# carlobaldassi/GaussDCA.jl

Hardware: AMD Instinct MI355X
Metric: end-to-end gDCA sec + achieved Cholesky TFLOP/s, N=500 M=50k q=21 (higher is better)
Workload: dtype f64

## Files before the change

gaussdca.jl_amd/csrc/gdca_api.hip:

```cpp
#include <algorithm>
#include <ctype.h>
#include <math.h>
#include <stdio.h>
#include <stdlib.h>
#include <string.h>
#include <strings.h>

#include "gdca_internal.h"
#include "gdca_launch.h"

#define MAX_EV 1024
#define N_SCRATCH 10

struct gdca_buf {
    void *p;
    size_t cap;
};

struct gdca_gate {
    hipEvent_t ev[4];
    int next, last, armed, refs;
    hipStream_t batch_stream;
};

// ... 609 lines not shown

static gdca_status member_error(gdca_ctx *lead, gdca_ctx *m, int k, gdca_status st)
{
    if (k > 0 && m != lead && m->err[0]) {
        char msg[sizeof(lead->err)];
        snprintf(msg, sizeof(msg), "member %d: %.400s", k, m->err);
        memcpy(lead->err, msg, sizeof(msg));
    }
    return st;
}

static gdca_status upload_done(gdca_ctx *ctx)
{
    HIPCHK(hipEventRecord(ctx->ev_upload, ctx->stream));
    HIPCHK(hipEventSynchronize(ctx->ev_upload));
    return GDCA_OK;
}

static double inverse_flops_model(double n)
{
    return (n * n * n / 3.0 + n * n / 2.0 + n / 6.0) + (2.0 * n * n * n / 3.0 + n * n / 2.0 + 5.0 * n / 6.0);
}

static int round_up(int x, int m)
{
    return (x + m - 1) / m * m;
}

static gdca_status weights_stage(gdca_ctx *ctx, const int8_t *Zd, int N, int M, int q, double theta_in, int fixed_thresh,
                                 bool want_theta_only, int mark_after_theta)
{
    hipStream_t s = ctx->stream;
    gdca_dev_scalars *sc = (gdca_dev_scalars *)ctx->sc.p;
    CHK(ensure(ctx, ctx->hist, (size_t)N * 32 * sizeof(uint32_t)));
    if (fixed_thresh >= 0) {
        gdca_launch_set_thresh(s, sc, fixed_thresh);
    } else {
        if (theta_in < 0.0) {
            gdca_fill_async(s, ctx->hist.p, 0, (size_t)N * 32 * sizeof(uint32_t));
            gdca_launch_column_hist(s, Zd, (uint32_t *)ctx->hist.p, N, M);
        }
        gdca_launch_theta_finalize(s, (const uint32_t *)ctx->hist.p, N, M, theta_in, sc);
    }
    CHK(check_launch(ctx, "theta"));
    if (mark_after_theta >= 0) CHK(mark(ctx, mark_after_theta));
    if (want_theta_only) return GDCA_OK;

    const int Mt = (M + GDCA_HTILE - 1) / GDCA_HTILE;
    CHK(ensure(ctx, ctx->Zb, gdca_bitplane_bytes(N, M)));
    CHK(ensure(ctx, ctx->hcnt, (size_t)Mt * GDCA_HTILE * sizeof(int32_t)));
    if (!ctx->tune.force_fallback && ctx->tune.hamming_mode != 0) CHK(ensure(ctx, ctx->hcand, gdca_hamming_cand_cap(M) * 8));
    const bool fp4 = !ctx->tune.force_fallback && ctx->tune.hamming_mode == 2;
    if (fp4) CHK(ensure(ctx, ctx->himg, gdca_fp4_image_bytes(N, M)));
    CHK(ensure(ctx, ctx->nk, (size_t)M * sizeof(int32_t)));
    CHK(ensure(ctx, ctx->W, (size_t)M * sizeof(double)));
    CHK(ensure(ctx, ctx->Wfix, (size_t)M * sizeof(unsigned long long)));
    gdca_fill_async(s, ctx->hcnt.p, 0, (size_t)Mt * GDCA_HTILE * sizeof(int32_t));
    gdca_launch_bitplane_pack(s, Zd, (uint32_t *)ctx->Zb.p, N, M, q, sc);
    if (ctx->tune.force_fallback)
        gdca_launch_hamming_fallback(s, Zd, (int32_t *)ctx->hcnt.p, N, M, sc);
    else
        gdca_launch_hamming(s, (const uint32_t *)ctx->Zb.p, Zd, (int32_t *)ctx->hcnt.p, N, M, sc, ctx->tune.hamming_mode, ctx->hcand.p, fp4 ? ctx->himg.p : nullptr);
    gdca_launch_weights(s, (const int32_t *)ctx->hcnt.p, M, gdca_fix_shift(M), (int32_t *)ctx->nk.p,
                        (double *)ctx->W.p, (unsigned long long *)ctx->Wfix.p);
    gdca_launch_meff(s, (const double *)ctx->W.p, M, sc);
    return check_launch(ctx, "weights");
}

static bool norm1_settled(const gdca_ctx *ctx, int N, int q, double pc)
{
    const double pi_cap = (1.0 - pc) + pc / (double)q;
    return pc > 0.0 && 2.0 * (double)N * pi_cap * (double)q * (double)q / pc <= ctx->tune.refine_cond && ctx->tune.refine != 1;
}

static gdca_status tally_stage(gdca_ctx *ctx, const int8_t *Zd, int N, int M, int q, const double *Meff_dev, double pc,
                               int mode, double *Pi_true_out, double *out, size_t ld, bool want_norm1 = false)
{
    hipStream_t s = ctx->stream;
    const int sdim = q - 1, n = N * sdim;
    const int shift = gdca_fix_shift(M);
    const int TJ = gdca_tally_tj(q, ctx->tune.tally_tj);
    const bool skip = gdca_tally_skip(q, TJ, ctx->tune.tally_skip, M);
    const size_t keep_list = (size_t)N * M * sizeof(uint32_t);
    if (skip) CHK(ensure(ctx, ctx->keep, keep_list + (size_t)N * sizeof(int) + N));
    CHK(ensure(ctx, ctx->Zt, (size_t)N * M));
    CHK(ensure(ctx, ctx->Zp, (size_t)round_up(N, 64) * M + 64));
    CHK(ensure(ctx, ctx->Pifix, (size_t)N * 32 * sizeof(unsigned long long)));
    CHK(ensure(ctx, ctx->Pipc, (size_t)n * sizeof(double)));
    gdca_launch_transpose_i8(s, Zd, (int8_t *)ctx->Zt.p, N, M);
    gdca_launch_colblock(s, Zd, (int8_t *)ctx->Zp.p, N, M, TJ);
    gdca_fill_async(s, ctx->Pifix.p, 0, (size_t)N * 32 * sizeof(unsigned long long));
    gdca_launch_pi_tally(s, Zd, (const unsigned long long *)ctx->Wfix.p, (unsigned long long *)ctx->Pifix.p, N, M, q,
                         (gdca_dev_scalars *)ctx->sc.p);
    gdca_launch_pi_finalize(s, (const unsigned long long *)ctx->Pifix.p, N, q, shift, Meff_dev, pc, Pi_true_out,
                            (double *)ctx->Pipc.p, want_norm1 ? &((gdca_dev_scalars *)ctx->sc.p)->pi_max : nullptr);
    const bool tm = want_norm1 && ctx->timing && ctx->n_ev >= 18;
    if (tm) CHK(mark(ctx, 9));
    uint32_t *keep = skip ? (uint32_t *)ctx->keep.p : nullptr;
    int *keep_n = skip ? (int *)((char *)ctx->keep.p + keep_list) : nullptr;
    uint8_t *sigma = skip ? (uint8_t *)(keep_n + N) : nullptr;
    if (skip)
        gdca_launch_tally_keep(s, (const int8_t *)ctx->Zt.p, (const unsigned long long *)ctx->Pifix.p, keep, keep_n, sigma, N, M, q);
    gdca_launch_pair_tally(s, (const int8_t *)ctx->Zp.p, (const int8_t *)ctx->Zt.p,
                           (const unsigned long long *)ctx->Wfix.p, N, M, q, shift, Meff_dev, pc,
                           (const double *)ctx->Pipc.p, mode, out, ld, TJ, keep, keep_n, sigma,
                           (const unsigned long long *)ctx->Pifix.p);
    if (tm) CHK(mark(ctx, 10));
    if (want_norm1 && !norm1_settled(ctx, N, q, pc))
        gdca_launch_cov_norm1(s, out, ld, N, q, pc, ctx->tune.refine_cond, (gdca_dev_scalars *)ctx->sc.p, ctx->tune.refine == 1);
    return check_launch(ctx, "tally");
}

static gdca_status inverse_job(gdca_ctx *ctx, int n, int n_pad, gdca_inverse_job *job)
{
    const size_t pbytes = (size_t)n_pad * GDCA_TILE * sizeof(double);
    const int nblk = n_pad / GDCA_TILE;
    const size_t sg = (size_t)4 * GDCA_TILE * 4 * GDCA_TILE * sizeof(double);
    const size_t fbytes = gdca_inverse_flag_bytes(n_pad);
    CHK(ensure(ctx, ctx->G, (size_t)8 * pbytes));
    CHK(ensure(ctx, ctx->H, (size_t)8 * pbytes));
    CHK(ensure(ctx, ctx->P, (size_t)GDCA_TILE * GDCA_TILE * sizeof(double)));
    CHK(ensure(ctx, ctx->Sg, 4 * sg + fbytes + (size_t)3 * (nblk + 2) * sizeof(int)));
    if (ctx->item0_cap < 3 * (nblk + 2)) {
        if (ctx->item0_host) HIPCHK(hipHostFree(ctx->item0_host));
        ctx->item0_host = nullptr;
        ctx->item0_cap = 0;
        HIPCHK(hipHostMalloc((void **)&ctx->item0_host, (size_t)3 * (nblk + 2) * sizeof(int), hipHostMallocDefault));
        ctx->item0_cap = 3 * (nblk + 2);
    }
    gdca_inverse_ws &ws = job->ws;
    for (int w = 0; w < 8; ++w) {
        ws.G[w] = (double *)((char *)ctx->G.p + (size_t)w * pbytes);
        ws.H[w] = (double *)((char *)ctx->H.p + (size_t)w * pbytes);
    }
    ws.P = (double *)ctx->P.p;
// ... 1812 lines not shown
```

gaussdca.jl_amd/csrc/gdca_internal.h:

```cpp
#pragma once

#include <hip/hip_runtime.h>
#include <stdint.h>

#include "gdca.h"

#define GDCA_TILE 128
#define GDCA_HTILE 128
#define GDCA_MAXQ 31
#define GDCA_STAMPS 20

struct gdca_dev_scalars {
    double theta;
    double Meff;
    unsigned long long pair_sum;
    int thresh;
    int info;
    int bad_symbol;
    int di_noconv;
    int ham_mode;
    int ham_cand;
    unsigned long long ham_ncand;
    unsigned long long sweep_cycles, sweep_ticks;
    double inv_norm1;
// ... 10 lines not shown
    int ramp;
    int ragged;
    int rem_tail;
    int panel_halves;
    int slab;
    int ring;
    int mcus;
    int mcu_solo;
    int sweep_debug;
    long sweep_timeout_ms;
    int sweep_retries;
    int tally_tj;
    int tally_skip;
    int hamming_mode;
    int force_fallback;
    int merge;
    int merge_blocks;
    int merge_mcus;
    int merge_group;
    int merge_tiles;
    int phased_fronts;
    int phased_grids;
    int phased_streams;
    int refine;
    double refine_cond;
    int cholesky;
    int energy_chunk;
    int pair_chunk;
    char sweep_trace[256];
};
void gdca_tuning_from_env(gdca_tuning *t);
bool gdca_tuning_set(gdca_tuning *t, const char *key, const char *value);

void gdca_launch_transpose_i8(hipStream_t s, const int8_t *Z, int8_t *Zt, int N, int M);
void gdca_launch_column_hist(hipStream_t s, const int8_t *Z, uint32_t *cnt, int N, int M);
void gdca_launch_theta_finalize(hipStream_t s, const uint32_t *cnt, int N, int M, double theta_in,
                                gdca_dev_scalars *sc);
void gdca_launch_set_thresh(hipStream_t s, gdca_dev_scalars *sc, int thresh);

size_t gdca_bitplane_bytes(int N, int M);
void gdca_launch_bitplane_pack(hipStream_t s, const int8_t *Z, uint32_t *Zb, int N, int M, int q,
                               gdca_dev_scalars *sc);
size_t gdca_hamming_cand_cap(int M);
size_t gdca_fp4_image_bytes(int N, int M);
void gdca_launch_hamming_fp4_probe(hipStream_t s, const uint32_t *Zb, int N, int M, int nprobe, gdca_dev_scalars *sc);
void gdca_launch_hamming_fp4(hipStream_t s, const uint32_t *Zb, void *img, int N, int M, gdca_dev_scalars *sc, void *cand_list, unsigned cap);
void gdca_launch_hamming(hipStream_t s, const uint32_t *Zb, const int8_t *Z, int32_t *cnt, int N, int M, gdca_dev_scalars *sc, int force,
                         void *cand_list, void *fp4_img);
void gdca_launch_hamming_fallback(hipStream_t s, const int8_t *Z, int32_t *cnt, int N, int M, const gdca_dev_scalars *sc);
void gdca_launch_weights(hipStream_t s, const int32_t *cnt, int M, int fix_shift, int32_t *n_out, double *W,
                         unsigned long long *Wfix);
void gdca_launch_meff(hipStream_t s, const double *W, int M, gdca_dev_scalars *sc);
void gdca_launch_fix_weights(hipStream_t s, const double *W, int M, int fix_shift, unsigned long long *Wfix,
                             gdca_dev_scalars *sc);
int gdca_fix_shift(int M);

void gdca_launch_pi_tally(hipStream_t s, const int8_t *Z, const unsigned long long *Wfix,
                          unsigned long long *Pifix, int N, int M, int q, gdca_dev_scalars *sc);
void gdca_launch_pi_finalize(hipStream_t s, const unsigned long long *Pifix, int N, int q, int fix_shift,
                             const double *Meff_dev, double pc, double *Pi_true, double *Pi_pc, double *pi_max = nullptr);
void gdca_launch_cov_norm1(hipStream_t s, const double *C, size_t ld, int N, int q, double pc, double cond_limit, gdca_dev_scalars *sc,
                           int always);
int gdca_tally_tj(int q, int tj_wanted);
void gdca_launch_colblock(hipStream_t s, const int8_t *Z, int8_t *Zc, int N, int M, int TJ);
bool gdca_tally_skip(int q, int TJ, int skip_wanted, int M);
void gdca_launch_tally_keep(hipStream_t s, const int8_t *Zt, const unsigned long long *Pifix, uint32_t *keep, int *keep_n,
                            uint8_t *sigma, int N, int M, int q);
void gdca_launch_pair_tally(hipStream_t s, const int8_t *Zc, const int8_t *Zt, const unsigned long long *Wfix,
                            int N, int M, int q, int fix_shift, const double *Meff_dev, double pc,
                            const double *Pi_pc, int mode, double *out, size_t ld, int TJ, const uint32_t *keep = nullptr,
                            const int *keep_n = nullptr, const uint8_t *sigma = nullptr, const unsigned long long *Pifix = nullptr);
void gdca_launch_cov_from_pij(hipStream_t s, const double *Pij, const double *Pi_pc, int N, int q, double pc, double *out, size_t ld);

void gdca_launch_add_pseudocount(hipStream_t s, const double *Pi_true, const double *Pij_true, int N, int q,
                                 double pc, double *Pi, double *Pij);
void gdca_launch_covariance(hipStream_t s, const double *Pi, const double *Pij, int n, double *C);
void gdca_launch_pad_identity(hipStream_t s, double *A, int n, int n_pad);
void gdca_launch_copy_in(hipStream_t s, const double *src, int n, double *dst, int n_pad);
void gdca_launch_copy_in_neg(hipStream_t s, const double *src, int n, double *dst, int n_pad);
void gdca_launch_copy_out_neg_sym(hipStream_t s, const double *A, int n_pad, double *dst, int n);
void gdca_launch_publish_scalars(hipStream_t s, const gdca_dev_scalars *sc, gdca_dev_scalars *host_mapped);
void gdca_launch_save_diag_blocks(hipStream_t s, const double *C, size_t ld, int N, int sdim, double *D);

struct gdca_inverse_ws {
    double *G[8];
    double *H[8];
    double *P;
    double *Sg[2];
    double *Pg[2];
    unsigned *flags;
    size_t flags_bytes;
    int *item0_host;
    const int *item0_host_dev;
    int *item0_dev;
    int update_cus;
};
struct gdca_inverse_job {
    double *A;
    int n_pad, n_real;
    gdca_inverse_ws ws;
// ... 53 lines not shown
```

gaussdca.jl_amd/csrc/k_tally.hip:

```cpp
#include "gdca_internal.h"
#include "gdca_launch.h"
#include <cstdlib>

typedef unsigned long long u64;

struct k_pi_tally_args {
    const int8_t *Z;
    const u64 *Wfix;
    u64 *Pifix;
    int N;
    int M;
    int seq_per_block;
    int q;
    gdca_dev_scalars *sc;
};
static inline k_pi_tally_args k_pi_tally_mk(const int8_t *Z, const u64 *Wfix, u64 *Pifix, int N, int M, int seq_per_block, int q, gdca_dev_scalars *sc)
{
    return k_pi_tally_args{Z, Wfix, Pifix, N, M, seq_per_block, q, sc};
}
template <int CAP>
__global__ __launch_bounds__(128) void k_pi_tally(const BatchArgs<k_pi_tally_args, CAP> B_)
{
    GDCA_MEMBER(B_);
    const int8_t *__restrict__ Z = a_.Z;
    const u64 *__restrict__ Wfix = a_.Wfix;
    u64 *__restrict__ Pifix = a_.Pifix;
    int N = a_.N;
    int M = a_.M;
    int seq_per_block = a_.seq_per_block;
    int q = a_.q;
    gdca_dev_scalars *sc = a_.sc;
    __shared__ u64 h[32][128];
    unsigned bad = 0;
    const int t = threadIdx.x;
    const int i = blockIdx.x * 128 + t;
#pragma unroll
    for (int z = 0; z < 32; ++z) h[z][t] = 0;
    const int kbeg = blockIdx.y * seq_per_block;
    const int kend = min(M, kbeg + seq_per_block);
    if (i < N) {
        const int8_t *p = Z + (size_t)kbeg * N + i;
        int k = kbeg;
        for (; k + 16 <= kend; k += 16) {
            int z[16];
#pragma unroll
            for (int u = 0; u < 16; ++u) {
                const unsigned raw = (uint8_t)p[(size_t)u * N];
                bad |= (raw - 1u) >= (unsigned)q;
                z[u] = raw & 31;
            }
#pragma unroll
            for (int u = 0; u < 16; ++u) h[z[u]][t] += Wfix[k + u];
            p += (size_t)16 * N;
        }
        for (; k < kend; ++k) {
            const unsigned raw = (uint8_t)p[0];
            bad |= (raw - 1u) >= (unsigned)q;
            h[raw & 31][t] += Wfix[k];
            p += N;
        }
        if (bad) atomicOr(&sc->bad_symbol, 1);
#pragma unroll
        for (int z = 0; z < 32; ++z) {
            const u64 v = h[z][t];
            if (v) atomicAdd(&Pifix[(size_t)i * 32 + z], v);
        }
    }
}

void gdca_launch_pi_tally(hipStream_t s, const int8_t *Z, const u64 *Wfix, u64 *Pifix, int N, int M, int q,
                          gdca_dev_scalars *sc)
{
    const int cb = (N + 127) / 128;
    int chunks = (512 + cb - 1) / cb;
    int spb = (M + chunks - 1) / chunks;
    if (spb < 64) spb = 64;
    chunks = (M + spb - 1) / spb;
    (gdca_launch<k_pi_tally_args, k_pi_tally<1>, k_pi_tally<GDCA_MAXB>>(dim3(cb, chunks), dim3(128), 0, s, k_pi_tally_mk(Z, Wfix, Pifix, N, M, spb, q, sc)));
}

struct k_pi_finalize_args {
    const u64 *Pifix;
    int N;
    int q;
    int fix_shift;
    const double *Meff_dev;
    double pc;
    double *Pi_true;
    double *Pi_pc;
    double *pi_max;
};
static inline k_pi_finalize_args k_pi_finalize_mk(const u64 *Pifix, int N, int q, int fix_shift, const double *Meff_dev, double pc, double *Pi_true, double *Pi_pc, double *pi_max)
{
    return k_pi_finalize_args{Pifix, N, q, fix_shift, Meff_dev, pc, Pi_true, Pi_pc, pi_max};
}
template <int CAP>
__global__ __launch_bounds__(256) void k_pi_finalize(const BatchArgs<k_pi_finalize_args, CAP> B_)
{
    GDCA_MEMBER(B_);
    const u64 *__restrict__ Pifix = a_.Pifix;
    int N = a_.N;
    int q = a_.q;
    int fix_shift = a_.fix_shift;
    const double *__restrict__ Meff_dev = a_.Meff_dev;
    double pc = a_.pc;
    double *__restrict__ Pi_true = a_.Pi_true;
    double *__restrict__ Pi_pc = a_.Pi_pc;
    double *__restrict__ pi_max = a_.pi_max;
    const int s = q - 1;
    const int e = blockIdx.x * 256 + threadIdx.x;
    double mine = 0.0;
// ... 43 lines not shown
    const double cheap = pc > 0.0 ? 2.0 * (double)N * sc->pi_max * (double)q * (double)q / pc : HUGE_VAL;
    if (!always && cheap <= cond_limit) return;
    __shared__ double red[256];
    double best = 0.0;
    for (int c = blockIdx.x; c < n; c += gridDim.x) {
        double a = 0.0;
        for (int r = threadIdx.x; r < n; r += 256) a += fabs(C[(size_t)r + (size_t)c * ld]);
        red[threadIdx.x] = a;
        __syncthreads();
        for (int w = 128; w > 0; w >>= 1) {
            if ((int)threadIdx.x < w) red[threadIdx.x] += red[threadIdx.x + w];
            __syncthreads();
        }
        best = fmax(best, red[0]);
        __syncthreads();
    }
    if (threadIdx.x == 0) atomicMax(reinterpret_cast<u64 *>(&sc->mat_norm1), (u64)__double_as_longlong(best));
}

void gdca_launch_cov_norm1(hipStream_t s, const double *C, size_t ld, int N, int q, double pc, double cond_limit, gdca_dev_scalars *sc, int always)
{
    (gdca_launch<k_cov_norm1_args, k_cov_norm1<1>, k_cov_norm1<GDCA_MAXB>>(dim3(512), dim3(256), 0, s, k_cov_norm1_mk(C, ld, N * (q - 1), N, q, pc, cond_limit, sc, always)));
}

void gdca_launch_pi_finalize(hipStream_t s, const u64 *Pifix, int N, int q, int fix_shift, const double *Meff_dev,
                             double pc, double *Pi_true, double *Pi_pc, double *pi_max)
{
    const int n = N * (q - 1);
    (gdca_launch<k_pi_finalize_args, k_pi_finalize<1>, k_pi_finalize<GDCA_MAXB>>(dim3((n + 255) / 256), dim3(256), 0, s, k_pi_finalize_mk(Pifix, N, q, fix_shift, Meff_dev, pc, Pi_true, Pi_pc, pi_max)));
}

#define TALLY_THREADS 1024
#define TALLY_CHUNK 1024

struct k_colblock_args {
    const int8_t *Z;
    int8_t *Zc;
    int N;
    int M;
    int TJ;
};
static inline k_colblock_args k_colblock_mk(const int8_t *Z, int8_t *Zc, int N, int M, int TJ)
{
    return k_colblock_args{Z, Zc, N, M, TJ};
}
template <int CAP>
__global__ __launch_bounds__(256) void k_colblock(const BatchArgs<k_colblock_args, CAP> B_)
{
    GDCA_MEMBER(B_);
    const int8_t *__restrict__ Z = a_.Z;
    int8_t *__restrict__ Zc = a_.Zc;
    int N = a_.N;
    int M = a_.M;
    int TJ = a_.TJ;
    __shared__ int8_t tile[64][64 + 4];
    const int k0 = blockIdx.y * 64, c0 = blockIdx.x * 64;
    const int tx = threadIdx.x & 63, ty = threadIdx.x >> 6;
#pragma unroll
    for (int r = 0; r < 16; ++r) {
        const int k = k0 + r * 4 + ty, c = c0 + tx;
        tile[r * 4 + ty][tx] = (k < M && c < N) ? Z[(size_t)k * N + c] : (int8_t)0;
    }
    __syncthreads();
    const int nb = 64 / TJ;
    for (int e = threadIdx.x; e < 64 * 64; e += 256) {
        const int blk = e / (64 * TJ), rem = e % (64 * TJ);
        const int kl = rem / TJ, cl = rem % TJ;
        const int k = k0 + kl;
        const int cb = c0 / TJ + blk;
        if (blk < nb && k < M && cb * TJ < ((N + TJ - 1) / TJ) * TJ)
            Zc[((size_t)cb * M + k) * TJ + cl] = tile[kl][blk * TJ + cl];
    }
}

void gdca_launch_colblock(hipStream_t s, const int8_t *Z, int8_t *Zc, int N, int M, int TJ)
{
    dim3 grid((N + 63) / 64, (M + 63) / 64);
    (gdca_launch<k_colblock_args, k_colblock<1>, k_colblock<GDCA_MAXB>>(grid, dim3(256), 0, s, k_colblock_mk(Z, Zc, N, M, TJ)));
}

#define KEEP_THREADS 256
#define KEEP_SLABS 16
struct k_tally_keep_args {
    const int8_t *Zt;
    const u64 *Pifix;
    uint32_t *keep;
    int *keep_n;
    uint8_t *sigma;
    int N;
    int M;
    int q;
};
static inline k_tally_keep_args k_tally_keep_mk(const int8_t *Zt, const u64 *Pifix, uint32_t *keep, int *keep_n, uint8_t *sigma, int N, int M, int q)
{
    return k_tally_keep_args{Zt, Pifix, keep, keep_n, sigma, N, M, q};
}
template <int CAP>
__global__ __launch_bounds__(KEEP_THREADS) void k_tally_keep(const BatchArgs<k_tally_keep_args, CAP> B_)
{
    GDCA_MEMBER(B_);
    const int8_t *__restrict__ Zt = a_.Zt;
    const u64 *__restrict__ Pifix = a_.Pifix;
    uint32_t *__restrict__ keep = a_.keep;
    int M = a_.M;
    int q = a_.q;
    constexpr int NW = KEEP_THREADS / 64;
    __shared__ unsigned wcnt[KEEP_SLABS * NW], woff[KEEP_SLABS * NW];
    const int i = blockIdx.x;
    const int t = threadIdx.x, lane = t & 63, wv = t >> 6;
    const u64 *P = Pifix + (size_t)i * 32;
    unsigned sig = 1;
    u64 best = P[1];
    for (int a = 2; a <= q; ++a) {
        const u64 v = P[a];
        if (v > best) {
            best = v;
            sig = (unsigned)a;
        }
    }
    const int8_t *zi = Zt + (size_t)i * M;
    uint32_t *out = keep + (size_t)i * M;
    const u64 lt = (1ull << lane) - 1ull;
    unsigned base = 0;
    for (int kc = 0; kc < M; kc += KEEP_THREADS * KEEP_SLABS) {
        unsigned raw[KEEP_SLABS], pos[KEEP_SLABS];
#pragma unroll
        for (int u = 0; u < KEEP_SLABS; ++u) {
            const int k = kc + u * KEEP_THREADS + t;
            raw[u] = k < M ? (unsigned)(uint8_t)zi[k] : 0u;
        }
#pragma unroll
        for (int u = 0; u < KEEP_SLABS; ++u) {
            const bool kp = (raw[u] - 1u) < (unsigned)q && raw[u] != sig;
            const u64 bal = __ballot(kp);
            pos[u] = kp ? (unsigned)__popcll(bal & lt) : ~0u;
            if (lane == 0) wcnt[u * NW + wv] = (unsigned)__popcll(bal);
        }
        __syncthreads();
        if (t < KEEP_SLABS * NW) {
            unsigned o = base;
            for (int e = 0; e < t; ++e) o += wcnt[e];
            woff[t] = o;
        }
        __syncthreads();
#pragma unroll
        for (int u = 0; u < KEEP_SLABS; ++u)
            if (pos[u] != ~0u) out[woff[u * NW + wv] + pos[u]] = ((unsigned)(kc + u * KEEP_THREADS + t) << 5) | raw[u];
        base = woff[KEEP_SLABS * NW - 1] + wcnt[KEEP_SLABS * NW - 1];
        __syncthreads();
    }
    if (t == 0) {
        a_.keep_n[i] = (int)base;
        a_.sigma[i] = (uint8_t)sig;
    }
}

void gdca_launch_tally_keep(hipStream_t s, const int8_t *Zt, const u64 *Pifix, uint32_t *keep, int *keep_n, uint8_t *sigma, int N, int M, int q)
{
    (gdca_launch<k_tally_keep_args, k_tally_keep<1>, k_tally_keep<GDCA_MAXB>>(dim3(N), dim3(KEEP_THREADS), 0, s, k_tally_keep_mk(Zt, Pifix, keep, keep_n, sigma, N, M, q)));
}

struct k_pair_tally_args {
    const int8_t *Zc;
    const int8_t *Zt;
    const u64 *Wfix;
    int N;
    int M;
    int q;
    int fix_shift;
    const double *Meff_dev;
    double pc;
    const double *Pi_pc;
    int mode;
    double *out;
    size_t ld;
    const uint32_t *keep;
    const int *keep_n;
    const uint8_t *sigma;
    const u64 *Pifix;
};
static inline k_pair_tally_args k_pair_tally_mk(const int8_t *Zc, const int8_t *Zt, const u64 *Wfix, int N, int M, int q, int fix_shift, const double *Meff_dev, double pc, const double *Pi_pc, int mode, double *out, size_t ld,
                                                const uint32_t *keep, const int *keep_n, const uint8_t *sigma, const u64 *Pifix)
{
    return k_pair_tally_args{Zc, Zt, Wfix, N, M, q, fix_shift, Meff_dev, pc, Pi_pc, mode, out, ld, keep, keep_n, sigma, Pifix};
}
template <int CAP, int TJ, bool SKIP>
__global__ __launch_bounds__(TALLY_THREADS) void k_pair_tally(const BatchArgs<k_pair_tally_args, CAP> B_)
{
    GDCA_MEMBER(B_);
    const int8_t *__restrict__ Zc = a_.Zc;
    const int8_t *__restrict__ Zt = a_.Zt;
    const u64 *__restrict__ Wfix = a_.Wfix;
    int N = a_.N;
// ... 248 lines not shown
```

gaussdca.jl_amd/csrc/k_theta.hip:

```cpp
#include "gdca_internal.h"
#include "gdca_launch.h"

struct k_transpose_i8_args {
    const int8_t *Z;
    int8_t *Zt;
    int N;
    int M;
};
static inline k_transpose_i8_args k_transpose_i8_mk(const int8_t *Z, int8_t *Zt, int N, int M)
{
    return k_transpose_i8_args{Z, Zt, N, M};
}
template <int CAP>
__global__ __launch_bounds__(256) void k_transpose_i8(const BatchArgs<k_transpose_i8_args, CAP> B_)
{
    GDCA_MEMBER(B_);
    const int8_t *__restrict__ Z = a_.Z;
    int8_t *__restrict__ Zt = a_.Zt;
    int N = a_.N;
    int M = a_.M;
    __shared__ int8_t tile[64][65];
    const int k0 = blockIdx.y * 64, i0 = blockIdx.x * 64;
    const int tx = threadIdx.x & 63, ty = threadIdx.x >> 6;
#pragma unroll
    for (int r = 0; r < 16; ++r) {
        const int k = k0 + r * 4 + ty, i = i0 + tx;
        tile[r * 4 + ty][tx] = (k < M && i < N) ? Z[(size_t)k * N + i] : (int8_t)0;
    }
    __syncthreads();
#pragma unroll
    for (int r = 0; r < 16; ++r) {
        const int i = i0 + r * 4 + ty, k = k0 + tx;
        if (i < N && k < M) Zt[(size_t)i * M + k] = tile[tx][r * 4 + ty];
    }
}

void gdca_launch_transpose_i8(hipStream_t s, const int8_t *Z, int8_t *Zt, int N, int M)
{
    dim3 grid((N + 63) / 64, (M + 63) / 64);
    (gdca_launch<k_transpose_i8_args, k_transpose_i8<1>, k_transpose_i8<GDCA_MAXB>>(grid, dim3(256), 0, s, k_transpose_i8_mk(Z, Zt, N, M)));
}

struct k_column_hist_args {
    const int8_t *Z;
    uint32_t *cnt;
    int N;
    int M;
    int seq_per_block;
};
static inline k_column_hist_args k_column_hist_mk(const int8_t *Z, uint32_t *cnt, int N, int M, int seq_per_block)
{
    return k_column_hist_args{Z, cnt, N, M, seq_per_block};
}
template <int CAP>
__global__ __launch_bounds__(256) void k_column_hist(const BatchArgs<k_column_hist_args, CAP> B_)
{
    GDCA_MEMBER(B_);
    const int8_t *__restrict__ Z = a_.Z;
    uint32_t *__restrict__ cnt = a_.cnt;
    int N = a_.N;
    int M = a_.M;
    int seq_per_block = a_.seq_per_block;
    __shared__ uint32_t h[32][256];
    const int t = threadIdx.x;
    const int i = blockIdx.x * 256 + t;
#pragma unroll
    for (int z = 0; z < 32; ++z) h[z][t] = 0;
    const int kbeg = blockIdx.y * seq_per_block;
    const int kend = min(M, kbeg + seq_per_block);
    if (i < N) {
        const int8_t *p = Z + (size_t)kbeg * N + i;
        int k = kbeg;
        for (; k + 16 <= kend; k += 16) {
            int z[16];
#pragma unroll
            for (int u = 0; u < 16; ++u) z[u] = p[(size_t)u * N] & 31;
#pragma unroll
            for (int u = 0; u < 16; ++u) h[z[u]][t] += 1;
            p += (size_t)16 * N;
        }
        for (; k < kend; ++k) {
            h[p[0] & 31][t] += 1;
            p += N;
        }
#pragma unroll
        for (int z = 0; z < 32; ++z) {
            const uint32_t v = h[z][t];
            if (v) atomicAdd(&cnt[(size_t)i * 32 + z], v);
        }
    }
}

void gdca_launch_column_hist(hipStream_t s, const int8_t *Z, uint32_t *cnt, int N, int M)
{
    const int cb = (N + 255) / 256;
    int chunks = (256 + cb - 1) / cb;
    int spb = (M + chunks - 1) / chunks;
    if (spb < 64) spb = 64;
    chunks = (M + spb - 1) / spb;
    (gdca_launch<k_column_hist_args, k_column_hist<1>, k_column_hist<GDCA_MAXB>>(dim3(cb, chunks), dim3(256), 0, s, k_column_hist_mk(Z, cnt, N, M, spb)));
}

struct k_theta_finalize_args {
    const uint32_t *cnt;
    int N;
    int M;
    double theta_in;
    gdca_dev_scalars *sc;
};
static inline k_theta_finalize_args k_theta_finalize_mk(const uint32_t *cnt, int N, int M, double theta_in, gdca_dev_scalars *sc)
{
    return k_theta_finalize_args{cnt, N, M, theta_in, sc};
}
template <int CAP>
__global__ __launch_bounds__(256) void k_theta_finalize(const BatchArgs<k_theta_finalize_args, CAP> B_)
{
    GDCA_MEMBER(B_);
    const uint32_t *__restrict__ cnt = a_.cnt;
    int N = a_.N;
    int M = a_.M;
    double theta_in = a_.theta_in;
    gdca_dev_scalars *sc = a_.sc;
    __shared__ unsigned long long red[256];
    double theta = theta_in;
    if (theta_in < 0.0) {
        unsigned long long acc = 0;
        for (int e = threadIdx.x; e < N * 32; e += 256) {
            const unsigned long long c = cnt[e];
            acc += c * (c - 1) / 2;
        }
        red[threadIdx.x] = acc;
        __syncthreads();
        for (int w = 128; w > 0; w >>= 1) {
// ... 52 lines not shown
```

Measured before the change: 45.97.

## Fuse relayout kernels, merge pi tally with keep-list build, deterministic column histogram

Transpose and column-block relayout now run as one kernel that reads each Z tile once. The pi tally and the keep-list construction are merged into one per-row kernel over the transposed Zt, using shared-memory atomics and ballot-based compaction. The column histogram now writes per-chunk partials with vectorized loads, and a separate sum kernel reduces them, which removes the memset and global atomics. This cuts launches and redundant passes over Z in the prologue, at the cost of extra scratch memory and a one-block-per-row pi kernel that may leave the GPU underused for small N.

```diff
diff --git a/gaussdca.jl_amd/csrc/gdca_api.hip b/gaussdca.jl_amd/csrc/gdca_api.hip
--- a/gaussdca.jl_amd/csrc/gdca_api.hip
+++ b/gaussdca.jl_amd/csrc/gdca_api.hip
@@ -665,14 +665,11 @@
 {
     hipStream_t s = ctx->stream;
     gdca_dev_scalars *sc = (gdca_dev_scalars *)ctx->sc.p;
-    CHK(ensure(ctx, ctx->hist, (size_t)N * 32 * sizeof(uint32_t)));
+    CHK(ensure(ctx, ctx->hist, gdca_column_hist_bytes(N, M)));
     if (fixed_thresh >= 0) {
         gdca_launch_set_thresh(s, sc, fixed_thresh);
     } else {
-        if (theta_in < 0.0) {
-            gdca_fill_async(s, ctx->hist.p, 0, (size_t)N * 32 * sizeof(uint32_t));
-            gdca_launch_column_hist(s, Zd, (uint32_t *)ctx->hist.p, N, M);
-        }
+        if (theta_in < 0.0) gdca_launch_column_hist(s, Zd, (uint32_t *)ctx->hist.p, N, M);
         gdca_launch_theta_finalize(s, (const uint32_t *)ctx->hist.p, N, M, theta_in, sc);
     }
     CHK(check_launch(ctx, "theta"));
@@ -716,24 +713,20 @@
     const bool skip = gdca_tally_skip(q, TJ, ctx->tune.tally_skip, M);
     const size_t keep_list = (size_t)N * M * sizeof(uint32_t);
     if (skip) CHK(ensure(ctx, ctx->keep, keep_list + (size_t)N * sizeof(int) + N));
-    CHK(ensure(ctx, ctx->Zt, (size_t)N * M));
+    CHK(ensure(ctx, ctx->Zt, (size_t)N * M + 3));
     CHK(ensure(ctx, ctx->Zp, (size_t)round_up(N, 64) * M + 64));
     CHK(ensure(ctx, ctx->Pifix, (size_t)N * 32 * sizeof(unsigned long long)));
     CHK(ensure(ctx, ctx->Pipc, (size_t)n * sizeof(double)));
-    gdca_launch_transpose_i8(s, Zd, (int8_t *)ctx->Zt.p, N, M);
-    gdca_launch_colblock(s, Zd, (int8_t *)ctx->Zp.p, N, M, TJ);
-    gdca_fill_async(s, ctx->Pifix.p, 0, (size_t)N * 32 * sizeof(unsigned long long));
-    gdca_launch_pi_tally(s, Zd, (const unsigned long long *)ctx->Wfix.p, (unsigned long long *)ctx->Pifix.p, N, M, q,
-                         (gdca_dev_scalars *)ctx->sc.p);
+    uint32_t *keep = skip ? (uint32_t *)ctx->keep.p : nullptr;
+    int *keep_n = skip ? (int *)((char *)ctx->keep.p + keep_list) : nullptr;
+    uint8_t *sigma = skip ? (uint8_t *)(keep_n + N) : nullptr;
+    gdca_launch_relayout(s, Zd, (int8_t *)ctx->Zt.p, (int8_t *)ctx->Zp.p, N, M, TJ);
+    gdca_launch_pi_keep(s, (const int8_t *)ctx->Zt.p, (const unsigned long long *)ctx->Wfix.p, (unsigned long long *)ctx->Pifix.p, keep, keep_n,
+                        sigma, N, M, q, (gdca_dev_scalars *)ctx->sc.p);
     gdca_launch_pi_finalize(s, (const unsigned long long *)ctx->Pifix.p, N, q, shift, Meff_dev, pc, Pi_true_out,
                             (double *)ctx->Pipc.p, want_norm1 ? &((gdca_dev_scalars *)ctx->sc.p)->pi_max : nullptr);
     const bool tm = want_norm1 && ctx->timing && ctx->n_ev >= 18;
     if (tm) CHK(mark(ctx, 9));
-    uint32_t *keep = skip ? (uint32_t *)ctx->keep.p : nullptr;
-    int *keep_n = skip ? (int *)((char *)ctx->keep.p + keep_list) : nullptr;
-    uint8_t *sigma = skip ? (uint8_t *)(keep_n + N) : nullptr;
-    if (skip)
-        gdca_launch_tally_keep(s, (const int8_t *)ctx->Zt.p, (const unsigned long long *)ctx->Pifix.p, keep, keep_n, sigma, N, M, q);
     gdca_launch_pair_tally(s, (const int8_t *)ctx->Zp.p, (const int8_t *)ctx->Zt.p,
                            (const unsigned long long *)ctx->Wfix.p, N, M, q, shift, Meff_dev, pc,
                            (const double *)ctx->Pipc.p, mode, out, ld, TJ, keep, keep_n, sigma,
diff --git a/gaussdca.jl_amd/csrc/gdca_internal.h b/gaussdca.jl_amd/csrc/gdca_internal.h
--- a/gaussdca.jl_amd/csrc/gdca_internal.h
+++ b/gaussdca.jl_amd/csrc/gdca_internal.h
@@ -66,7 +66,8 @@
 void gdca_tuning_from_env(gdca_tuning *t);
 bool gdca_tuning_set(gdca_tuning *t, const char *key, const char *value);
 
-void gdca_launch_transpose_i8(hipStream_t s, const int8_t *Z, int8_t *Zt, int N, int M);
+void gdca_launch_relayout(hipStream_t s, const int8_t *Z, int8_t *Zt, int8_t *Zc, int N, int M, int TJ);
+size_t gdca_column_hist_bytes(int N, int M);
 void gdca_launch_column_hist(hipStream_t s, const int8_t *Z, uint32_t *cnt, int N, int M);
 void gdca_launch_theta_finalize(hipStream_t s, const uint32_t *cnt, int N, int M, double theta_in,
                                 gdca_dev_scalars *sc);
@@ -89,17 +90,14 @@
                              gdca_dev_scalars *sc);
 int gdca_fix_shift(int M);
 
-void gdca_launch_pi_tally(hipStream_t s, const int8_t *Z, const unsigned long long *Wfix,
-                          unsigned long long *Pifix, int N, int M, int q, gdca_dev_scalars *sc);
+void gdca_launch_pi_keep(hipStream_t s, const int8_t *Zt, const unsigned long long *Wfix, unsigned long long *Pifix, uint32_t *keep,
+                         int *keep_n, uint8_t *sigma, int N, int M, int q, gdca_dev_scalars *sc);
 void gdca_launch_pi_finalize(hipStream_t s, const unsigned long long *Pifix, int N, int q, int fix_shift,
                              const double *Meff_dev, double pc, double *Pi_true, double *Pi_pc, double *pi_max = nullptr);
 void gdca_launch_cov_norm1(hipStream_t s, const double *C, size_t ld, int N, int q, double pc, double cond_limit, gdca_dev_scalars *sc,
                            int always);
 int gdca_tally_tj(int q, int tj_wanted);
-void gdca_launch_colblock(hipStream_t s, const int8_t *Z, int8_t *Zc, int N, int M, int TJ);
 bool gdca_tally_skip(int q, int TJ, int skip_wanted, int M);
-void gdca_launch_tally_keep(hipStream_t s, const int8_t *Zt, const unsigned long long *Pifix, uint32_t *keep, int *keep_n,
-                            uint8_t *sigma, int N, int M, int q);
 void gdca_launch_pair_tally(hipStream_t s, const int8_t *Zc, const int8_t *Zt, const unsigned long long *Wfix,
                             int N, int M, int q, int fix_shift, const double *Meff_dev, double pc,
                             const double *Pi_pc, int mode, double *out, size_t ld, int TJ, const uint32_t *keep = nullptr,
diff --git a/gaussdca.jl_amd/csrc/k_tally.hip b/gaussdca.jl_amd/csrc/k_tally.hip
--- a/gaussdca.jl_amd/csrc/k_tally.hip
+++ b/gaussdca.jl_amd/csrc/k_tally.hip
@@ -4,79 +4,183 @@
 
 typedef unsigned long long u64;
 
-struct k_pi_tally_args {
-    const int8_t *Z;
+#define PIK_THREADS 512
+#define PIK_SLABS 4
+struct k_pi_keep_args {
+    const int8_t *Zt;
     const u64 *Wfix;
     u64 *Pifix;
+    uint32_t *keep;
+    int *keep_n;
+    uint8_t *sigma;
     int N;
     int M;
-    int seq_per_block;
     int q;
     gdca_dev_scalars *sc;
 };
-static inline k_pi_tally_args k_pi_tally_mk(const int8_t *Z, const u64 *Wfix, u64 *Pifix, int N, int M, int seq_per_block, int q, gdca_dev_scalars *sc)
-{
-    return k_pi_tally_args{Z, Wfix, Pifix, N, M, seq_per_block, q, sc};
+static inline k_pi_keep_args k_pi_keep_mk(const int8_t *Zt, const u64 *Wfix, u64 *Pifix, uint32_t *keep, int *keep_n, uint8_t *sigma, int N, int M, int q, gdca_dev_scalars *sc)
+{
+    return k_pi_keep_args{Zt, Wfix, Pifix, keep, keep_n, sigma, N, M, q, sc};
 }
 template <int CAP>
-__global__ __launch_bounds__(128) void k_pi_tally(const BatchArgs<k_pi_tally_args, CAP> B_)
+__global__ __launch_bounds__(PIK_THREADS) void k_pi_keep(const BatchArgs<k_pi_keep_args, CAP> B_)
 {
     GDCA_MEMBER(B_);
-    const int8_t *__restrict__ Z = a_.Z;
     const u64 *__restrict__ Wfix = a_.Wfix;
     u64 *__restrict__ Pifix = a_.Pifix;
-    int N = a_.N;
+    uint32_t *__restrict__ keep = a_.keep;
     int M = a_.M;
-    int seq_per_block = a_.seq_per_block;
     int q = a_.q;
     gdca_dev_scalars *sc = a_.sc;
-    __shared__ u64 h[32][128];
+    constexpr int NW = PIK_THREADS / 64;
+    constexpr int NC = PIK_SLABS * NW;
+    static_assert(PIK_THREADS >= 256 && NC <= 64, "the fold below takes 256 threads; one wave scans the counts");
+    __shared__ u64 bins[32 * 64];
+    __shared__ u64 tot[32];
+    __shared__ unsigned wcnt[2][NC], woff[2][NC + 1];
+    const int i = blockIdx.x;
+    const int t = threadIdx.x, lane = t & 63, wv = t >> 6;
+    const int8_t *zi = a_.Zt + (size_t)i * M;
+    const int off = (int)(reinterpret_cast<uintptr_t>(zi) & 3);
+    const uint32_t *__restrict__ zw = reinterpret_cast<const uint32_t *>(zi - off);
+    const int D = (off + M + 3) >> 2;
+    const bool wpair = off == 0 && (reinterpret_cast<uintptr_t>(Wfix) & 15) == 0;
+    for (int e = t; e < 32 * 64; e += PIK_THREADS) bins[e] = 0;
+    __syncthreads();
     unsigned bad = 0;
-    const int t = threadIdx.x;
-    const int i = blockIdx.x * 128 + t;
-#pragma unroll
-    for (int z = 0; z < 32; ++z) h[z][t] = 0;
-    const int kbeg = blockIdx.y * seq_per_block;
-    const int kend = min(M, kbeg + seq_per_block);
-    if (i < N) {
-        const int8_t *p = Z + (size_t)kbeg * N + i;
-        int k = kbeg;
-        for (; k + 16 <= kend; k += 16) {
-            int z[16];
-#pragma unroll
-            for (int u = 0; u < 16; ++u) {
-                const unsigned raw = (uint8_t)p[(size_t)u * N];
-                bad |= (raw - 1u) >= (unsigned)q;
-                z[u] = raw & 31;
-            }
-#pragma unroll
-            for (int u = 0; u < 16; ++u) h[z[u]][t] += Wfix[k + u];
-            p += (size_t)16 * N;
-        }
-        for (; k < kend; ++k) {
-            const unsigned raw = (uint8_t)p[0];
-            bad |= (raw - 1u) >= (unsigned)q;
-            h[raw & 31][t] += Wfix[k];
-            p += N;
-        }
-        if (bad) atomicOr(&sc->bad_symbol, 1);
-#pragma unroll
-        for (int z = 0; z < 32; ++z) {
-            const u64 v = h[z][t];
-            if (v) atomicAdd(&Pifix[(size_t)i * 32 + z], v);
-        }
-    }
-}
-
-void gdca_launch_pi_tally(hipStream_t s, const int8_t *Z, const u64 *Wfix, u64 *Pifix, int N, int M, int q,
-                          gdca_dev_scalars *sc)
-{
-    const int cb = (N + 127) / 128;
-    int chunks = (512 + cb - 1) / cb;
-    int spb = (M + chunks - 1) / chunks;
-    if (spb < 64) spb = 64;
-    chunks = (M + spb - 1) / spb;
-    (gdca_launch<k_pi_tally_args, k_pi_tally<1>, k_pi_tally<GDCA_MAXB>>(dim3(cb, chunks), dim3(128), 0, s, k_pi_tally_mk(Z, Wfix, Pifix, N, M, spb, q, sc)));
+    for (int d0 = 0; d0 < D; d0 += PIK_THREADS * PIK_SLABS) {
+        uint32_t z[PIK_SLABS];
+        u64 w[PIK_SLABS][4];
+#pragma unroll
+        for (int u = 0; u < PIK_SLABS; ++u) {
+            const int d = d0 + u * PIK_THREADS + t;
+            const int k = 4 * d - off;
+            z[u] = 0;
+#pragma unroll
+            for (int j = 0; j < 4; ++j) w[u][j] = 0;
+            if (d < D) {
+                z[u] = zw[d];
+                if (wpair && k + 3 < M) {
+                    const ulonglong2 w0 = reinterpret_cast<const ulonglong2 *>(Wfix + k)[0];
+                    const ulonglong2 w1 = reinterpret_cast<const ulonglong2 *>(Wfix + k)[1];
+                    w[u][0] = w0.x;
+                    w[u][1] = w0.y;
+                    w[u][2] = w1.x;
+                    w[u][3] = w1.y;
+                } else {
+#pragma unroll
+                    for (int j = 0; j < 4; ++j)
+                        if ((unsigned)(k + j) < (unsigned)M) w[u][j] = Wfix[k + j];
+                }
+            }
+        }
+#pragma unroll
+        for (int u = 0; u < PIK_SLABS; ++u) {
+            const int d = d0 + u * PIK_THREADS + t;
+            const int k = 4 * d - off;
+            if (d < D) {
+#pragma unroll
+                for (int j = 0; j < 4; ++j) {
+                    if ((unsigned)(k + j) < (unsigned)M) {
+                        const unsigned raw = (z[u] >> (8 * j)) & 255u;
+                        bad |= (raw - 1u) >= (unsigned)q;
+                        atomicAdd(&bins[(raw & 31u) * 64 + lane], w[u][j]);
+                    }
+                }
+            }
+        }
+    }
+    if (bad) atomicOr(&sc->bad_symbol, 1);
+    __syncthreads();
+    if (t < 256) {
+        const int z = t >> 3, part = t & 7;
+        u64 v = 0;
+#pragma unroll
+        for (int e = 0; e < 8; ++e) v += bins[z * 64 + part * 8 + e];
+        v += __shfl_xor(v, 1, 64);
+        v += __shfl_xor(v, 2, 64);
+        v += __shfl_xor(v, 4, 64);
+        if (part == 0) {
+            tot[z] = v;
+            Pifix[(size_t)i * 32 + z] = v;
+        }
+    }
+    if (keep == nullptr) return;
+    __syncthreads();
+    unsigned sig = 1;
+    u64 best = tot[1];
+    for (int a = 2; a <= q; ++a) {
+        const u64 v = tot[a];
+        if (v > best) {
+            best = v;
+            sig = (unsigned)a;
+        }
+    }
+    uint32_t *out = keep + (size_t)i * M;
+    const u64 lt = (1ull << lane) - 1ull;
+    unsigned base = 0;
+    int par = 0;
+    for (int d0 = 0; d0 < D; d0 += PIK_THREADS * PIK_SLABS, par ^= 1) {
+        uint32_t z[PIK_SLABS];
+        unsigned kpm[PIK_SLABS], pos[PIK_SLABS];
+#pragma unroll
+        for (int u = 0; u < PIK_SLABS; ++u) {
+            const int d = d0 + u * PIK_THREADS + t;
+            z[u] = d < D ? zw[d] : 0u;
+        }
+#pragma unroll
+        for (int u = 0; u < PIK_SLABS; ++u) {
+            const int d = d0 + u * PIK_THREADS + t;
+            const int k = 4 * d - off;
+            unsigned m = 0, pre = 0, cnt = 0;
+#pragma unroll
+            for (int j = 0; j < 4; ++j) {
+                const unsigned raw = (z[u] >> (8 * j)) & 255u;
+                const bool kp = d < D && (unsigned)(k + j) < (unsigned)M && (raw - 1u) < (unsigned)q && raw != sig;
+                const u64 bal = __ballot(kp);
+                pre += (unsigned)__popcll(bal & lt);
+                cnt += (unsigned)__popcll(bal);
+                m |= (kp ? 1u : 0u) << j;
+            }
+            kpm[u] = m;
+            pos[u] = pre;
+            if (lane == 0) wcnt[par][u * NW + wv] = cnt;
+        }
+        __syncthreads();
+        if (wv == 0) {
+            const unsigned v = lane < NC ? wcnt[par][lane] : 0u;
+            unsigned incl = v;
+#pragma unroll
+            for (int o = 1; o < NC; o <<= 1) {
+                const unsigned nb = __shfl_up(incl, o, 64);
+                if (lane >= o) incl += nb;
+            }
+            if (lane < NC) woff[par][lane] = base + incl - v;
+            if (lane == NC - 1) woff[par][NC] = base + incl;
+        }
+        __syncthreads();
+#pragma unroll
+        for (int u = 0; u < PIK_SLABS; ++u) {
+            if (kpm[u]) {
+                const int k = 4 * (d0 + u * PIK_THREADS + t) - off;
+                unsigned o = woff[par][u * NW + wv] + pos[u];
+#pragma unroll
+                for (int j = 0; j < 4; ++j)
+                    if ((kpm[u] >> j) & 1u) out[o++] = ((unsigned)(k + j) << 5) | ((z[u] >> (8 * j)) & 255u);
+            }
+        }
+        base = woff[par][NC];
+    }
+    if (t == 0) {
+        a_.keep_n[i] = (int)base;
+        a_.sigma[i] = (uint8_t)sig;
+    }
+}
+
+void gdca_launch_pi_keep(hipStream_t s, const int8_t *Zt, const u64 *Wfix, u64 *Pifix, uint32_t *keep, int *keep_n, uint8_t *sigma, int N, int M,
+                         int q, gdca_dev_scalars *sc)
+{
+    (gdca_launch<k_pi_keep_args, k_pi_keep<1>, k_pi_keep<GDCA_MAXB>>(dim3(N, 1), dim3(PIK_THREADS), 0, s, k_pi_keep_mk(Zt, Wfix, Pifix, keep, keep_n, sigma, N, M, q, sc)));
 }
 
 struct k_pi_finalize_args {
@@ -186,133 +290,6 @@
 
 #define TALLY_THREADS 1024
 #define TALLY_CHUNK 1024
-
-struct k_colblock_args {
-    const int8_t *Z;
-    int8_t *Zc;
-    int N;
-    int M;
-    int TJ;
-};
-static inline k_colblock_args k_colblock_mk(const int8_t *Z, int8_t *Zc, int N, int M, int TJ)
-{
-    return k_colblock_args{Z, Zc, N, M, TJ};
-}
-template <int CAP>
-__global__ __launch_bounds__(256) void k_colblock(const BatchArgs<k_colblock_args, CAP> B_)
-{
-    GDCA_MEMBER(B_);
-    const int8_t *__restrict__ Z = a_.Z;
-    int8_t *__restrict__ Zc = a_.Zc;
-    int N = a_.N;
-    int M = a_.M;
-    int TJ = a_.TJ;
-    __shared__ int8_t tile[64][64 + 4];
-    const int k0 = blockIdx.y * 64, c0 = blockIdx.x * 64;
-    const int tx = threadIdx.x & 63, ty = threadIdx.x >> 6;
-#pragma unroll
-    for (int r = 0; r < 16; ++r) {
-        const int k = k0 + r * 4 + ty, c = c0 + tx;
-        tile[r * 4 + ty][tx] = (k < M && c < N) ? Z[(size_t)k * N + c] : (int8_t)0;
-    }
-    __syncthreads();
-    const int nb = 64 / TJ;
-    for (int e = threadIdx.x; e < 64 * 64; e += 256) {
-        const int blk = e / (64 * TJ), rem = e % (64 * TJ);
-        const int kl = rem / TJ, cl = rem % TJ;
-        const int k = k0 + kl;
-        const int cb = c0 / TJ + blk;
-        if (blk < nb && k < M && cb * TJ < ((N + TJ - 1) / TJ) * TJ)
-            Zc[((size_t)cb * M + k) * TJ + cl] = tile[kl][blk * TJ + cl];
-    }
-}
-
-void gdca_launch_colblock(hipStream_t s, const int8_t *Z, int8_t *Zc, int N, int M, int TJ)
-{
-    dim3 grid((N + 63) / 64, (M + 63) / 64);
-    (gdca_launch<k_colblock_args, k_colblock<1>, k_colblock<GDCA_MAXB>>(grid, dim3(256), 0, s, k_colblock_mk(Z, Zc, N, M, TJ)));
-}
-
-#define KEEP_THREADS 256
-#define KEEP_SLABS 16
-struct k_tally_keep_args {
-    const int8_t *Zt;
-    const u64 *Pifix;
-    uint32_t *keep;
-    int *keep_n;
-    uint8_t *sigma;
-    int N;
-    int M;
-    int q;
-};
-static inline k_tally_keep_args k_tally_keep_mk(const int8_t *Zt, const u64 *Pifix, uint32_t *keep, int *keep_n, uint8_t *sigma, int N, int M, int q)
-{
-    return k_tally_keep_args{Zt, Pifix, keep, keep_n, sigma, N, M, q};
-}
-template <int CAP>
-__global__ __launch_bounds__(KEEP_THREADS) void k_tally_keep(const BatchArgs<k_tally_keep_args, CAP> B_)
-{
-    GDCA_MEMBER(B_);
-    const int8_t *__restrict__ Zt = a_.Zt;
-    const u64 *__restrict__ Pifix = a_.Pifix;
-    uint32_t *__restrict__ keep = a_.keep;
-    int M = a_.M;
-    int q = a_.q;
-    constexpr int NW = KEEP_THREADS / 64;
-    __shared__ unsigned wcnt[KEEP_SLABS * NW], woff[KEEP_SLABS * NW];
-    const int i = blockIdx.x;
-    const int t = threadIdx.x, lane = t & 63, wv = t >> 6;
-    const u64 *P = Pifix + (size_t)i * 32;
-    unsigned sig = 1;
-    u64 best = P[1];
-    for (int a = 2; a <= q; ++a) {
-        const u64 v = P[a];
-        if (v > best) {
-            best = v;
-            sig = (unsigned)a;
-        }
-    }
-    const int8_t *zi = Zt + (size_t)i * M;
-    uint32_t *out = keep + (size_t)i * M;
-    const u64 lt = (1ull << lane) - 1ull;
-    unsigned base = 0;
-    for (int kc = 0; kc < M; kc += KEEP_THREADS * KEEP_SLABS) {
-        unsigned raw[KEEP_SLABS], pos[KEEP_SLABS];
-#pragma unroll
-        for (int u = 0; u < KEEP_SLABS; ++u) {
-            const int k = kc + u * KEEP_THREADS + t;
-            raw[u] = k < M ? (unsigned)(uint8_t)zi[k] : 0u;
-        }
-#pragma unroll
-        for (int u = 0; u < KEEP_SLABS; ++u) {
-            const bool kp = (raw[u] - 1u) < (unsigned)q && raw[u] != sig;
-            const u64 bal = __ballot(kp);
-            pos[u] = kp ? (unsigned)__popcll(bal & lt) : ~0u;
-            if (lane == 0) wcnt[u * NW + wv] = (unsigned)__popcll(bal);
-        }
-        __syncthreads();
-        if (t < KEEP_SLABS * NW) {
-            unsigned o = base;
-            for (int e = 0; e < t; ++e) o += wcnt[e];
-            woff[t] = o;
-        }
-        __syncthreads();
-#pragma unroll
-        for (int u = 0; u < KEEP_SLABS; ++u)
-            if (pos[u] != ~0u) out[woff[u * NW + wv] + pos[u]] = ((unsigned)(kc + u * KEEP_THREADS + t) << 5) | raw[u];
-        base = woff[KEEP_SLABS * NW - 1] + wcnt[KEEP_SLABS * NW - 1];
-        __syncthreads();
-    }
-    if (t == 0) {
-        a_.keep_n[i] = (int)base;
-        a_.sigma[i] = (uint8_t)sig;
-    }
-}
-
-void gdca_launch_tally_keep(hipStream_t s, const int8_t *Zt, const u64 *Pifix, uint32_t *keep, int *keep_n, uint8_t *sigma, int N, int M, int q)
-{
-    (gdca_launch<k_tally_keep_args, k_tally_keep<1>, k_tally_keep<GDCA_MAXB>>(dim3(N), dim3(KEEP_THREADS), 0, s, k_tally_keep_mk(Zt, Pifix, keep, keep_n, sigma, N, M, q)));
-}
 
 struct k_pair_tally_args {
     const int8_t *Zc;
diff --git a/gaussdca.jl_amd/csrc/k_theta.hip b/gaussdca.jl_amd/csrc/k_theta.hip
--- a/gaussdca.jl_amd/csrc/k_theta.hip
+++ b/gaussdca.jl_amd/csrc/k_theta.hip
@@ -1,104 +1,230 @@
 #include "gdca_internal.h"
 #include "gdca_launch.h"
 
-struct k_transpose_i8_args {
+struct k_relayout_args {
     const int8_t *Z;
     int8_t *Zt;
+    int8_t *Zc;
     int N;
     int M;
-};
-static inline k_transpose_i8_args k_transpose_i8_mk(const int8_t *Z, int8_t *Zt, int N, int M)
-{
-    return k_transpose_i8_args{Z, Zt, N, M};
-}
-template <int CAP>
-__global__ __launch_bounds__(256) void k_transpose_i8(const BatchArgs<k_transpose_i8_args, CAP> B_)
+    int TJ;
+};
+static inline k_relayout_args k_relayout_mk(const int8_t *Z, int8_t *Zt, int8_t *Zc, int N, int M, int TJ)
+{
+    return k_relayout_args{Z, Zt, Zc, N, M, TJ};
+}
+template <int CAP>
+__global__ __launch_bounds__(256) void k_relayout(const BatchArgs<k_relayout_args, CAP> B_)
 {
     GDCA_MEMBER(B_);
     const int8_t *__restrict__ Z = a_.Z;
     int8_t *__restrict__ Zt = a_.Zt;
+    int8_t *__restrict__ Zc = a_.Zc;
     int N = a_.N;
     int M = a_.M;
-    __shared__ int8_t tile[64][65];
-    const int k0 = blockIdx.y * 64, i0 = blockIdx.x * 64;
-    const int tx = threadIdx.x & 63, ty = threadIdx.x >> 6;
-#pragma unroll
-    for (int r = 0; r < 16; ++r) {
-        const int k = k0 + r * 4 + ty, i = i0 + tx;
-        tile[r * 4 + ty][tx] = (k < M && i < N) ? Z[(size_t)k * N + i] : (int8_t)0;
+    int TJ = a_.TJ;
+    __shared__ uint32_t tile[64][17];
+    const int k0 = blockIdx.y * 64, c0 = blockIdx.x * 64;
+    const int t = threadIdx.x;
+    if (((N & 3) == 0) && ((reinterpret_cast<uintptr_t>(Z) & 3) == 0)) {
+        const int d = t & 15, c = c0 + 4 * d;
+#pragma unroll
+        for (int r = 0; r < 4; ++r) {
+            const int kl = r * 16 + (t >> 4), k = k0 + kl;
+            uint32_t v = 0;
+            if (k < M && c < N) v = *reinterpret_cast<const uint32_t *>(Z + (size_t)k * N + c);
+            tile[kl][d] = v;
+        }
+    } else {
+        uint8_t *tb = reinterpret_cast<uint8_t *>(&tile[0][0]);
+        const int tx = t & 63, ty = t >> 6;
+#pragma unroll
+        for (int r = 0; r < 16; ++r) {
+            const int kl = r * 4 + ty, k = k0 + kl, c = c0 + tx;
+            tb[kl * 68 + tx] = (k < M && c < N) ? (uint8_t)Z[(size_t)k * N + c] : (uint8_t)0;
+        }
     }
     __syncthreads();
-#pragma unroll
-    for (int r = 0; r < 16; ++r) {
-        const int i = i0 + r * 4 + ty, k = k0 + tx;
-        if (i < N && k < M) Zt[(size_t)i * M + k] = tile[tx][r * 4 + ty];
-    }
-}
-
-void gdca_launch_transpose_i8(hipStream_t s, const int8_t *Z, int8_t *Zt, int N, int M)
+    {
+        const int q16 = TJ >> 4;
+        const int blk = t / (64 * q16), rem = t % (64 * q16);
+        const int kl = rem / q16, h = rem % q16;
+        const int k = k0 + kl, cb = c0 / TJ + blk;
+        if (k < M && cb * TJ < N) {
+            const int d0 = blk * (TJ >> 2) + 4 * h;
+            const uint4 v = make_uint4(tile[kl][d0], tile[kl][d0 + 1], tile[kl][d0 + 2], tile[kl][d0 + 3]);
+            *reinterpret_cast<uint4 *>(Zc + ((size_t)cb * M + k) * TJ + 16 * h) = v;
+        }
+    }
+    {
+        const bool wide = ((M & 3) == 0) && ((reinterpret_cast<uintptr_t>(Zt) & 3) == 0);
+        const int bk = t & 15, bc = t >> 4;
+        uint32_t r[4];
+#pragma unroll
+        for (int j = 0; j < 4; ++j) r[j] = tile[4 * bk + j][bc];
+        const int k = k0 + 4 * bk;
+#pragma unroll
+        for (int j = 0; j < 4; ++j) {
+            const int i = c0 + 4 * bc + j;
+            const uint32_t o = ((r[0] >> (8 * j)) & 255u) | (((r[1] >> (8 * j)) & 255u) << 8) | (((r[2] >> (8 * j)) & 255u) << 16) |
+                               (((r[3] >> (8 * j)) & 255u) << 24);
+            if (i < N && k < M) {
+                int8_t *dst = Zt + (size_t)i * M + k;
+                if (wide) {
+                    *reinterpret_cast<uint32_t *>(dst) = o;
+                } else {
+#pragma unroll
+                    for (int e = 0; e < 4; ++e)
+                        if (k + e < M) dst[e] = (int8_t)((o >> (8 * e)) & 255u);
+                }
+            }
+        }
+    }
+}
+
+void gdca_launch_relayout(hipStream_t s, const int8_t *Z, int8_t *Zt, int8_t *Zc, int N, int M, int TJ)
 {
     dim3 grid((N + 63) / 64, (M + 63) / 64);
-    (gdca_launch<k_transpose_i8_args, k_transpose_i8<1>, k_transpose_i8<GDCA_MAXB>>(grid, dim3(256), 0, s, k_transpose_i8_mk(Z, Zt, N, M)));
-}
-
+    (gdca_launch<k_relayout_args, k_relayout<1>, k_relayout<GDCA_MAXB>>(grid, dim3(256), 0, s, k_relayout_mk(Z, Zt, Zc, N, M, TJ)));
+}
+
+#define HIST_THREADS 1024
+#define HIST_ROWS 8
 struct k_column_hist_args {
     const int8_t *Z;
-    uint32_t *cnt;
+    uint32_t *out;
     int N;
     int M;
     int seq_per_block;
 };
-static inline k_column_hist_args k_column_hist_mk(const int8_t *Z, uint32_t *cnt, int N, int M, int seq_per_block)
-{
-    return k_column_hist_args{Z, cnt, N, M, seq_per_block};
-}
-template <int CAP>
-__global__ __launch_bounds__(256) void k_column_hist(const BatchArgs<k_column_hist_args, CAP> B_)
+static inline k_column_hist_args k_column_hist_mk(const int8_t *Z, uint32_t *out, int N, int M, int seq_per_block)
+{
+    return k_column_hist_args{Z, out, N, M, seq_per_block};
+}
+template <int CAP>
+__global__ __launch_bounds__(HIST_THREADS) void k_column_hist(const BatchArgs<k_column_hist_args, CAP> B_)
 {
     GDCA_MEMBER(B_);
     const int8_t *__restrict__ Z = a_.Z;
-    uint32_t *__restrict__ cnt = a_.cnt;
+    uint32_t *__restrict__ out = a_.out;
     int N = a_.N;
     int M = a_.M;
     int seq_per_block = a_.seq_per_block;
-    __shared__ uint32_t h[32][256];
-    const int t = threadIdx.x;
-    const int i = blockIdx.x * 256 + t;
-#pragma unroll
-    for (int z = 0; z < 32; ++z) h[z][t] = 0;
+    constexpr int NW = HIST_THREADS / 64;
+    static_assert(HIST_THREADS >= 512, "the store of the counts takes 512 threads");
+    __shared__ __attribute__((aligned(16))) uint32_t h[32 * 256];
+    const int t = threadIdx.x, lane = t & 63, wv = t >> 6;
+    for (int e = t; e < 32 * 256; e += HIST_THREADS) h[e] = 0;
+    const int c = blockIdx.x * 256 + 4 * lane;
+    const int nv = N - c < 4 ? N - c : 4;
     const int kbeg = blockIdx.y * seq_per_block;
     const int kend = min(M, kbeg + seq_per_block);
-    if (i < N) {
-        const int8_t *p = Z + (size_t)kbeg * N + i;
-        int k = kbeg;
-        for (; k + 16 <= kend; k += 16) {
-            int z[16];
-#pragma unroll
-            for (int u = 0; u < 16; ++u) z[u] = p[(size_t)u * N] & 31;
-#pragma unroll
-            for (int u = 0; u < 16; ++u) h[z[u]][t] += 1;
-            p += (size_t)16 * N;
-        }
-        for (; k < kend; ++k) {
-            h[p[0] & 31][t] += 1;
-            p += N;
-        }
-#pragma unroll
-        for (int z = 0; z < 32; ++z) {
-            const uint32_t v = h[z][t];
-            if (v) atomicAdd(&cnt[(size_t)i * 32 + z], v);
-        }
-    }
-}
-
-void gdca_launch_column_hist(hipStream_t s, const int8_t *Z, uint32_t *cnt, int N, int M)
-{
-    const int cb = (N + 255) / 256;
-    int chunks = (256 + cb - 1) / cb;
+    const bool wide = ((N & 3) == 0) && ((reinterpret_cast<uintptr_t>(Z) & 3) == 0);
+    __syncthreads();
+    if (nv > 0) {
+        for (int k = kbeg + wv; k < kend; k += NW * HIST_ROWS) {
+            uint32_t v[HIST_ROWS];
+#pragma unroll
+            for (int u = 0; u < HIST_ROWS; ++u) {
+                const int ku = k + u * NW;
+                v[u] = 0;
+                if (ku < kend) {
+                    const int8_t *p = Z + (size_t)ku * N + c;
+                    if (wide) {
+                        v[u] = *reinterpret_cast<const uint32_t *>(p);
+                    } else {
+#pragma unroll
+                        for (int j = 0; j < 4; ++j)
+                            if (j < nv) v[u] |= (uint32_t)(uint8_t)p[j] << (8 * j);
+                    }
+                }
+            }
+#pragma unroll
+            for (int u = 0; u < HIST_ROWS; ++u) {
+                if (k + u * NW < kend) {
+#pragma unroll
+                    for (int j = 0; j < 4; ++j)
+                        if (j < nv) atomicAdd(&h[((v[u] >> (8 * j)) & 31u) * 256 + j * 64 + lane], 1u);
+                }
+            }
+        }
+    }
+    __syncthreads();
+    {
+        const int x = t & 255, half = t >> 8;
+        const int l = x & 63, j = x >> 6;
+        const int col = blockIdx.x * 256 + 4 * l + j;
+        if (t < 512 && col < N) {
+            uint32_t *dst = out + ((size_t)blockIdx.y * N + col) * 32 + 16 * half;
+#pragma unroll
+            for (int g = 0; g < 4; ++g) {
+                const int z = 16 * half + 4 * g;
+                const uint4 o = make_uint4(h[z * 256 + j * 64 + l], h[(z + 1) * 256 + j * 64 + l], h[(z + 2) * 256 + j * 64 + l],
+                                           h[(z + 3) * 256 + j * 64 + l]);
+                reinterpret_cast<uint4 *>(dst)[g] = o;
+            }
+        }
+    }
+}
+
+struct k_column_hist_sum_args {
+    const uint32_t *part;
+    uint32_t *cnt;
+    int total;
+    int chunks;
+};
+static inline k_column_hist_sum_args k_column_hist_sum_mk(const uint32_t *part, uint32_t *cnt, int total, int chunks)
+{
+    return k_column_hist_sum_args{part, cnt, total, chunks};
+}
+template <int CAP>
+__global__ __launch_bounds__(256) void k_column_hist_sum(const BatchArgs<k_column_hist_sum_args, CAP> B_)
+{
+    GDCA_MEMBER(B_);
+    const uint32_t *__restrict__ part = a_.part;
+    uint32_t *__restrict__ cnt = a_.cnt;
+    int total = a_.total;
+    int chunks = a_.chunks;
+    const int e = blockIdx.x * 256 + threadIdx.x;
+    if (e >= total) return;
+    uint32_t acc = 0;
+    int c = 0;
+    for (; c + 8 <= chunks; c += 8) {
+        uint32_t v[8];
+#pragma unroll
+        for (int u = 0; u < 8; ++u) v[u] = part[(size_t)(c + u) * total + e];
+#pragma unroll
+        for (int u = 0; u < 8; ++u) acc += v[u];
+    }
+    for (; c < chunks; ++c) acc += part[(size_t)c * total + e];
+    cnt[e] = acc;
+}
+
+static int column_hist_split(int N, int M, int *spb_out)
+{
+    const int strips = (N + 255) / 256;
+    int chunks = (256 + strips - 1) / strips;
     int spb = (M + chunks - 1) / chunks;
     if (spb < 64) spb = 64;
     chunks = (M + spb - 1) / spb;
-    (gdca_launch<k_column_hist_args, k_column_hist<1>, k_column_hist<GDCA_MAXB>>(dim3(cb, chunks), dim3(256), 0, s, k_column_hist_mk(Z, cnt, N, M, spb)));
+    if (spb_out) *spb_out = spb;
+    return chunks;
+}
+
+size_t gdca_column_hist_bytes(int N, int M)
+{
+    const int chunks = column_hist_split(N, M, nullptr);
+    return (size_t)N * 32 * sizeof(uint32_t) * (size_t)(chunks > 1 ? 1 + chunks : 1);
+}
+
+void gdca_launch_column_hist(hipStream_t s, const int8_t *Z, uint32_t *cnt, int N, int M)
+{
+    int spb;
+    const int chunks = column_hist_split(N, M, &spb);
+    uint32_t *out = chunks > 1 ? cnt + (size_t)N * 32 : cnt;
+    (gdca_launch<k_column_hist_args, k_column_hist<1>, k_column_hist<GDCA_MAXB>>(dim3((N + 255) / 256, chunks), dim3(HIST_THREADS), 0, s, k_column_hist_mk(Z, out, N, M, spb)));
+    if (chunks > 1)
+        (gdca_launch<k_column_hist_sum_args, k_column_hist_sum<1>, k_column_hist_sum<GDCA_MAXB>>(dim3((N * 32 + 255) / 256, 1), dim3(256), 0, s, k_column_hist_sum_mk(out, cnt, N * 32, chunks)));
 }
 
 struct k_theta_finalize_args {
```

New measurement: 46.66 (median of 6 runs). 1.5% higher.
